# kaspanet/rusty-kaspa

Hardware: NVIDIA H100
Metric: schnorr_sig_verifies_per_sec (higher is better)
Workload: dtype u32 limbs (256-bit modular integer)

## Files before the change

__graft_entry__.py:

```python
import os
import subprocess
import sys

ROOT = os.path.dirname(os.path.abspath(__file__))
CSRC = os.path.join(ROOT, "rusty_kaspa_b200", "csrc")
LIB = os.path.join(ROOT, "rusty_kaspa_b200", "libkgv.so")
NVCC_FLAGS = ["-gencode", "arch=compute_90a,code=sm_90a", "-O3", "-lineinfo", "-std=c++17", "-shared", "-Xcompiler", "-fPIC"]


def _newer(target, sources):
    if not os.path.exists(target):
        return True
    t = os.path.getmtime(target)
    return any(os.path.getmtime(s) > t for s in sources)


def _run(cmd, **kw):
    r = subprocess.run(cmd, capture_output=True, text=True, **kw)
    if r.returncode != 0:
        raise RuntimeError("command failed: %s\n%s\n%s" % (" ".join(cmd), r.stdout[-4000:], r.stderr[-4000:]))
    return r


def build():
    srcs = [os.path.join(d, f) for d, _, fs in os.walk(CSRC) for f in fs] + [os.path.join(ROOT, "include", "kgv.h")]
    units = sorted(s for s in srcs if s.endswith(".cu") or s.endswith(".cpp"))
    if _newer(LIB, srcs):
        nvcc = os.environ.get("NVCC", "nvcc")
        _run([nvcc] + NVCC_FLAGS + ["-o", LIB] + units)
    _run(["make", "-C", os.path.join(ROOT, "oracle")])
    hs = os.path.join(ROOT, "tests", "hostsim")
    for name in ("hostsim_arith", "hostsim_secp", "hostsim_comb", "hostsim_joint", "hostsim_hash", "hostsim_u3072", "hostsim_script"):
        src, out = os.path.join(hs, name + ".cpp"), os.path.join(hs, "lib" + name + ".so")
        if os.path.exists(src) and _newer(out, [src] + srcs):
            _run(["g++", "-O2", "-std=c++17", "-shared", "-fPIC", "-o", out, src])
    sg_src, sg_lib = os.path.join(ROOT, "tools", "simgen", "kgv_simgen.cpp"), os.path.join(ROOT, "tools", "simgen", "libkgv_simgen.so")
    if os.path.exists(sg_src) and _newer(sg_lib, [sg_src]):
        _run(["g++", "-O2", "-std=c++17", "-shared", "-fPIC", "-o", sg_lib, sg_src])
    for name in ("host_mirror_test", "script_engine_mirror_test"):
        cpp_src, cpp_bin = os.path.join(ROOT, "tests", "cpp", name + ".cpp"), os.path.join(ROOT, "tests", "cpp", name)
        if os.path.exists(cpp_src) and _newer(cpp_bin, [cpp_src, LIB, os.path.join(ROOT, "include", "kgv.hpp"), os.path.join(ROOT, "include", "kgv.h")]):
            _run(["g++", "-O2", "-std=c++17", "-o", cpp_bin, cpp_src, "-L" + os.path.join(ROOT, "rusty_kaspa_b200"), "-l:libkgv.so", "-Wl,-rpath,$ORIGIN/../../rusty_kaspa_b200"])
    sys.path.insert(0, ROOT)
    import rusty_kaspa_b200
    from rusty_kaspa_b200 import _lib
    _lib.load()


def smoke():
    import ctypes
    import numpy as np
    sys.path.insert(0, ROOT)
    import rusty_kaspa_b200 as rk
    from rusty_kaspa_b200 import workload as W
    pk, msg, sig, kind = W.schnorr_triples(4096, seed=7, n_keys=256, n_nonces=256, frac_bitflip=0.05, frac_adversarial=0.05)
    ctx = rk.GpuContext(0)
    got = ctx.verify_schnorr_batch(pk, msg, sig)
    ora = ctypes.CDLL(os.path.join(ROOT, "oracle", "libkaspa_oracle.so"))
    ora.ok_secp_init()
    exp = np.zeros(len(pk), dtype=np.uint8)
    vp = lambda a: a.ctypes.data_as(ctypes.c_void_p)
    ora.ok_schnorr_verify_batch(vp(pk), vp(msg), vp(sig), ctypes.c_size_t(len(pk)), vp(exp), 4)
    assert (got == exp).all(), "GPU verdicts differ from the oracle"
    assert (got[kind == 0] == 1).all() and not (got[kind != 0] == 1).any()
    bm = ctx.status_to_bitmap(got)
# ... 43 lines not shown
```

rusty_kaspa_b200/csrc/kgv_internal.h:

```cpp
#pragma once
#include <cuda_runtime.h>
#include <cstdint>
#include <mutex>
#include <string>
#include <thread>
#include <vector>

#ifndef KGV_BLOCK
#define KGV_BLOCK 128
#endif
#ifndef KGV_BLOCKS_PER_SM
#define KGV_BLOCKS_PER_SM 3
#endif

#ifndef KGV_ITEMS
#define KGV_ITEMS 4
#endif

struct kgv_ctx {
  int device = 0;
  cudaStream_t own_stream = nullptr;
  cudaStream_t aux_stream = nullptr;
  cudaEvent_t ev_fork = nullptr, ev_join = nullptr;
  cudaEvent_t ev_time[3] = {};
  cudaEvent_t ev_chunk[32] = {};
  cudaStream_t stream = nullptr;
  uint32_t* gtab = nullptr;
  uint8_t* d_in = nullptr;
  size_t d_in_cap = 0;
  uint8_t* d_out = nullptr;
  size_t d_out_cap = 0;
  uint8_t* d_batch = nullptr;
  size_t d_batch_cap = 0;
  struct PrefetchSlot {
    uint8_t* buf = nullptr;
    size_t cap = 0;
    bool valid = false;
    const void *txs = nullptr, *inputs = nullptr, *outputs = nullptr, *entries = nullptr, *bytes = nullptr;
    size_t n_txs = 0, n_inputs = 0, n_outputs = 0, n_bytes = 0;
    cudaEvent_t done = nullptr;
    std::thread worker;
    int rc = 0;
    std::string err;
  } prefetch[2];
  int prefetch_next = 0;
  cudaEvent_t ev_prefetch = nullptr;
  cudaStream_t copy_stream = nullptr;
  uint8_t* d_scratch = nullptr;
  size_t d_scratch_cap = 0;
  uint8_t* d_work = nullptr;
  size_t d_work_cap = 0;
  uint8_t* d_replay = nullptr;
  size_t d_replay_cap = 0;
  uint8_t* d_keys[2] = {};
  size_t d_keys_cap[2] = {};
  uint8_t* d_mu = nullptr;
  size_t d_mu_cap = 0;
  struct {
    bool valid = false;
    const void *txs = nullptr, *inputs = nullptr, *outputs = nullptr, *bytes = nullptr;
    size_t nt = 0, ni = 0, no = 0, n_blocks = 0;
    size_t o_ids = 0, o_itx = 0, o_otx = 0, o_ent = 0, o_acc = 0, o_txb = 0, o_rng = 0;
    size_t o_src = 0, o_inf = 0, o_apv = 0;
  } last_replay;
  struct kgv_sigcache* sigcache = nullptr;
  struct kgv_comm* shard_comm = nullptr;
  std::vector<uint8_t*> parked;
  uint64_t launches = 0;
  uint32_t last_script_rounds = 0;
  struct {
    size_t n = 0;
    unsigned blocks = 0;
    bool key_cache = false;
    cudaStream_t stream = nullptr;
  } last_verify[2];
  int resident_blocks = 132 * KGV_BLOCKS_PER_SM;
  std::recursive_mutex mu;
  std::string err;
};

int kgv_ptr_is_device(const void* p);
int kgv_malloc(kgv_ctx* ctx, void** p, size_t bytes);
int kgv_reserve(kgv_ctx* ctx, uint8_t** buf, size_t* cap, size_t need);

#include "../../include/kgv.h"
struct kgv_dev_batch {
  const kgv_tx* txs;
  const kgv_input* inputs;
// ... 44 lines not shown
```

rusty_kaspa_b200/csrc/kgv_lib.cu:

```cuda
#include "../../include/kgv.h"
#include "kgv_internal.h"
#include "kgv_verify.cuh"
#include "kgv_lanes.cuh"

#include <cuda_runtime.h>
#include <cstdio>
#include <algorithm>
#include <cstring>
#include <mutex>
#include <string>

using namespace kgv;

struct SmemTab {
  uint32_t* base;
  __device__ __forceinline__ void put(int e, int w, uint32_t v) { base[(e * 16 + w) * KGV_BLOCK] = v; }
  __device__ __forceinline__ uint32_t get(int e, int w) const { return base[(e * 16 + w) * KGV_BLOCK]; }
  __device__ __forceinline__ uint4* chunk(int q) const { return reinterpret_cast<uint4*>(base - threadIdx.x) + q * KGV_BLOCK + threadIdx.x; }
};
__device__ __forceinline__ void stage_fetch(SmemTab& tab, int s, const uint32_t* entry) {
#pragma unroll
  for (int c = 0; c < 4; c++) {
    const uint32_t dst = (uint32_t)__cvta_generic_to_shared(tab.chunk(4 * s + c));
    asm volatile("cp.async.cg.shared.global [%0], [%1], 16;" ::"r"(dst), "l"(entry + 4 * c) : "memory");
// ... 129 lines not shown
      bool eq = true;
      for (int k = 0; k < nw; k++) eq = eq && v[k] == w[k];
      if (eq) break;
    }
    s = (s + 1) & mask;
  }
  const uint32_t act = __activemask(), ball = __ballot_sync(act, won);
  const int lane = threadIdx.x & 31, leader = __ffs(act) - 1;
  uint32_t base = 0;
  if (lane == leader && ball) base = atomicAdd(n_rec, (uint32_t)__popc(ball));
  base = __shfl_sync(act, base, leader);
  if (won) {
    const uint32_t r = base + __popc(ball & ((1u << lane) - 1));
    if (key_form(r + 1, n) != KGV_KEYS_INLINE) {
      rec_rep[r] = (uint32_t)i;
      table[s].rec = r + 1;
    }
  }
  item_slot[i] = s;
}

template <bool ECDSA>
__global__ void __launch_bounds__(KGV_BLOCK, KGV_BLOCKS_PER_SM) k_key_prepare(const uint8_t* __restrict__ pk, size_t n_arg, const uint32_t* __restrict__ n_dev,
                                                                              const uint32_t* __restrict__ rec_rep, const uint32_t* __restrict__ n_rec,
                                                                              uint32_t* __restrict__ recs) {
  const size_t n = n_dev ? (size_t)*n_dev : n_arg;
  const uint32_t r = blockIdx.x * blockDim.x + threadIdx.x;
  const int f = key_form(*n_rec, n);
  if (r >= *n_rec || f == KGV_KEYS_INLINE) return;
  uint32_t w[9];
  key_words<false, ECDSA>(w, pk, rec_rep[r]);
  if (f == KGV_KEYS_COMB) {
    uint32_t* rec = recs + (size_t)r * KGV_KJ_WORDS;
    key_comb_build(rec, ECDSA ? w[8] : 2u, w);
    if (rec[KGV_KC_STATUS] == KGV_ST_VALID) key_joint_build(rec);
  } else key_rec_build(recs + (size_t)r * KGV_KR_WORDS, ECDSA ? w[8] : 2u, w);
}

template <bool ECDSA>
__device__ __forceinline__ void batch_mul(fe& r, const fe& a, const fe& b) {
  if constexpr (ECDSA) sc_mul(r.v, a.v, b.v);
  else fe_mul(r, a, b);
}
template <bool ECDSA, bool ALIGNED, bool INDEXED>
__device__ __forceinline__ void verify_body(const uint8_t* __restrict__ pk, const uint8_t* __restrict__ msg, const uint8_t* __restrict__ sig,
                                            size_t n_arg, uint8_t* __restrict__ status, const uint32_t* __restrict__ gtab,
                                            const uint32_t* __restrict__ index, const uint32_t* __restrict__ n_dev, KeyCacheView kc) {
  extern __shared__ uint32_t smem[];
  const size_t n = (INDEXED && n_dev) ? (size_t)*n_dev : n_arg;
  const size_t total = (size_t)gridDim.x * KGV_BLOCK;
  const size_t tid = (size_t)blockIdx.x * KGV_BLOCK + threadIdx.x;
  SmemTab tab{smem + threadIdx.x};
  fe X[KGV_ITEMS], Y[KGV_ITEMS], RX[KGV_ITEMS], D[KGV_ITEMS], pre[KGV_ITEMS], M[KGV_ITEMS];
  const uint32_t* KR[KGV_ITEMS];
  bool comb = false;
  uint8_t st[KGV_ITEMS];
#pragma unroll 1
  for (size_t base = 0; base < n; base += total * KGV_ITEMS) {
  fe acc;
  fe_set_u32(acc, 1);
  bool any = false;
#pragma unroll 1
  for (int j = 0; j < KGV_ITEMS; j++) {
    size_t i = base + tid + (size_t)j * total;
    st[j] = KGV_ST_INVALID;
    if (i >= n) continue;
    if (INDEXED) i = index[i];
    uint32_t pkw[9], mw[8], sw[16];
    key_words<ALIGNED, ECDSA>(pkw, pk, i);
    load_be32<ALIGNED>(mw, msg + 32 * i);
    load_be32<ALIGNED>(sw, sig + 64 * i);
    load_be32<ALIGNED>(sw + 8, sig + 64 * i + 32);
    const KeySrc key = kc.key_of(i, n);
    fe x, y, rx, d, m;
    uint8_t s1;
    if constexpr (ECDSA) s1 = ecdsa_phase1(x, y, rx.v, d.v, m.v, pkw[8], pkw, mw, sw, key);
    else s1 = schnorr_phase1(x, y, d, rx, pkw, mw, sw, tab, gtab, GLoadDev(), key);
    st[j] = s1;
    if (s1 == KGV_ST_PENDING) {
      X[j] = x; Y[j] = y; RX[j] = rx; D[j] = d;
      if constexpr (ECDSA) { M[j] = m; KR[j] = key.rec; comb = key.comb; }
      pre[j] = acc;
      batch_mul<ECDSA>(acc, acc, d);
      any = true;
    }
  }
  if (any) {
    fe inv;
    if constexpr (ECDSA) sc_inv(inv.v, acc.v);
    else fe_inv(inv, acc);
#pragma unroll 1
    for (int j = KGV_ITEMS - 1; j >= 0; j--) {
      if (st[j] != KGV_ST_PENDING) continue;
      fe di;
      batch_mul<ECDSA>(di, inv, pre[j]);
      batch_mul<ECDSA>(inv, inv, D[j]);
      if constexpr (ECDSA) st[j] = ecdsa_phase2(X[j], Y[j], RX[j].v, di.v, M[j].v, tab, gtab, GLoadDev(), KeySrc{KR[j], comb});
      else st[j] = schnorr_phase2(X[j], Y[j], di, RX[j]);
    }
  }
#pragma unroll 1
  for (int j = 0; j < KGV_ITEMS; j++) {
    size_t i = base + tid + (size_t)j * total;
    if (i < n) status[INDEXED ? index[i] : i] = st[j];
  }
  }
}

template <bool ALIGNED, bool INDEXED>
__global__ void __launch_bounds__(KGV_BLOCK, KGV_BLOCKS_PER_SM)
k_schnorr_verify(const uint8_t* __restrict__ pk, const uint8_t* __restrict__ msg, const uint8_t* __restrict__ sig, size_t n_arg,
                 uint8_t* __restrict__ status, const uint32_t* __restrict__ gtab, const uint32_t* __restrict__ index, const uint32_t* __restrict__ n_dev,
                 KeyCacheView kc) {
  verify_body<false, ALIGNED, INDEXED>(pk, msg, sig, n_arg, status, gtab, index, n_dev, kc);
}
template <bool ALIGNED, bool INDEXED>
__global__ void __launch_bounds__(KGV_BLOCK, KGV_BLOCKS_PER_SM)
k_ecdsa_verify(const uint8_t* __restrict__ pk, const uint8_t* __restrict__ msg, const uint8_t* __restrict__ sig, size_t n_arg,
               uint8_t* __restrict__ status, const uint32_t* __restrict__ gtab, const uint32_t* __restrict__ index, const uint32_t* __restrict__ n_dev,
               KeyCacheView kc) {
  verify_body<true, ALIGNED, INDEXED>(pk, msg, sig, n_arg, status, gtab, index, n_dev, kc);
}
using VerifyKernel = void (*)(const uint8_t*, const uint8_t*, const uint8_t*, size_t, uint8_t*, const uint32_t*, const uint32_t*, const uint32_t*,
                              KeyCacheView);
static const VerifyKernel k_verify[2][2][2] = {
    {{k_schnorr_verify<false, false>, k_schnorr_verify<true, false>}, {k_schnorr_verify<false, true>, k_schnorr_verify<true, true>}},
    {{k_ecdsa_verify<false, false>, k_ecdsa_verify<true, false>}, {k_ecdsa_verify<false, true>, k_ecdsa_verify<true, true>}}};

struct DevTrace {
  uint32_t* out;
  __device__ __forceinline__ void operator()(int stage, const uint32_t* w, int n) const {
    for (int i = 0; i < n && i < 16; i++) out[stage * 16 + i] = w[i];
  }
};
__global__ void __launch_bounds__(KGV_BLOCK, KGV_BLOCKS_PER_SM)
k_schnorr_trace(const uint8_t* __restrict__ pk, const uint8_t* __restrict__ msg, const uint8_t* __restrict__ sig,
                uint8_t* __restrict__ status, const uint32_t* __restrict__ gtab, uint32_t* __restrict__ dbg) {
  extern __shared__ uint32_t smem[];
  if (threadIdx.x != 0 || blockIdx.x != 0) return;
  uint32_t pkw[8], mw[8], sw[16];
  load_be32<false>(pkw, pk);
  load_be32<false>(mw, msg);
  load_be32<false>(sw, sig);
  load_be32<false>(sw + 8, sig + 32);
  SmemTab tab{smem + threadIdx.x};
  status[0] = schnorr_verify_core(pkw, mw, sw, tab, gtab, GLoadDev(), DevTrace{dbg});
}

__global__ void k_selftest(int op, const uint32_t* __restrict__ in, uint32_t* __restrict__ out, int n) {
  int i = blockIdx.x * blockDim.x + threadIdx.x;
  if (i >= n) return;
  uint32_t a[8], b[8], r[16];
#pragma unroll
  for (int k = 0; k < 8; k++) { a[k] = in[i * 16 + k]; b[k] = in[i * 16 + 8 + k]; }
#pragma unroll
  for (int k = 0; k < 16; k++) r[k] = 0;
  fe fa, fb, fr;
// ... 113 lines not shown
    CK(cudaEventCreateWithFlags(&ctx->ev_join, cudaEventDisableTiming));
    CK(cudaMalloc((void**)&ctx->gtab, (size_t)8 * 65536 * 16 * sizeof(uint32_t)));
    k_build_gtab<<<(8 * 65536) / 128, 128, 0, ctx->stream>>>(ctx->gtab);
    CK(cudaGetLastError());
    ctx->launches++;
    const int smem = KGV_BLOCK * 128 * (int)sizeof(uint32_t);
    for (const auto& kind : k_verify)
      for (const auto& form : kind)
        for (VerifyKernel k : form) CK(cudaFuncSetAttribute(k, cudaFuncAttributeMaxDynamicSharedMemorySize, smem));
    int per_sm = 0, sms = 0;
    CK(cudaOccupancyMaxActiveBlocksPerMultiprocessor(&per_sm, k_verify[0][0][1], KGV_BLOCK, smem));
    CK(cudaDeviceGetAttribute(&sms, cudaDevAttrMultiProcessorCount, device));
    ctx->resident_blocks = per_sm * sms > 0 ? per_sm * sms : 132 * KGV_BLOCKS_PER_SM;
    CK(cudaStreamSynchronize(ctx->stream));
    return KGV_OK;
  };
  int rc = body();
  if (rc != KGV_OK) {
    fprintf(stderr, "kgv_create: %s\n", ctx->err.c_str());
    delete ctx;
    return rc;
  }
  *out = ctx;
  return KGV_OK;
}

extern "C" void kgv_destroy(kgv_ctx* ctx) {
  if (!ctx) return;
  cudaSetDevice(ctx->device);
  for (auto& P : ctx->prefetch) if (P.worker.joinable()) P.worker.join();
  if (ctx->copy_stream) cudaStreamSynchronize(ctx->copy_stream);
  cudaStreamSynchronize(ctx->stream);
  if (ctx->gtab) cudaFree(ctx->gtab);
  for (uint8_t* b : {ctx->d_in, ctx->d_out, ctx->d_batch, ctx->prefetch[0].buf, ctx->prefetch[1].buf, ctx->d_scratch, ctx->d_mu, ctx->d_work, ctx->d_replay, ctx->d_keys[0], ctx->d_keys[1]})
    if (b) cudaFree(b);
  for (uint8_t* b : ctx->parked) cudaFree(b);
  for (cudaEvent_t e : ctx->ev_chunk) if (e) cudaEventDestroy(e);
  for (cudaEvent_t e : ctx->ev_time) if (e) cudaEventDestroy(e);
  if (ctx->ev_prefetch) cudaEventDestroy(ctx->ev_prefetch);
  for (auto& P : ctx->prefetch) if (P.done) cudaEventDestroy(P.done);
  if (ctx->copy_stream) cudaStreamDestroy(ctx->copy_stream);
  if (ctx->ev_fork) cudaEventDestroy(ctx->ev_fork);
  if (ctx->ev_join) cudaEventDestroy(ctx->ev_join);
  if (ctx->aux_stream) cudaStreamDestroy(ctx->aux_stream);
  if (ctx->own_stream) cudaStreamDestroy(ctx->own_stream);
  delete ctx;
}

extern "C" int kgv_set_stream(kgv_ctx* ctx, void* cuda_stream) {
  if (!ctx) return KGV_ERR_ARG;
  std::lock_guard<std::recursive_mutex> g(ctx->mu);
  ctx->stream = (cudaStream_t)cuda_stream;
  return KGV_OK;
}

extern "C" int kgv_reset_stream(kgv_ctx* ctx) {
  if (!ctx) return KGV_ERR_ARG;
  std::lock_guard<std::recursive_mutex> g(ctx->mu);
  ctx->stream = ctx->own_stream;
  return KGV_OK;
}

extern "C" int kgv_synchronize(kgv_ctx* ctx) {
  if (!ctx) return KGV_ERR_ARG;
  std::lock_guard<std::recursive_mutex> g(ctx->mu);
  CK(cudaSetDevice(ctx->device));
  CK(cudaStreamSynchronize(ctx->stream));
// ... 20 lines not shown
  const size_t o_rep = (o_item + n * 4 + 255) & ~(size_t)255, o_rec = (o_rep + (size_t)cap * 4 + 255) & ~(size_t)255;
  int rc = kgv_reserve(ctx, &ctx->d_keys[ecdsa], &ctx->d_keys_cap[ecdsa], o_rec + rec_bytes);
  if (rc) return rc;
  uint8_t* K = ctx->d_keys[ecdsa];
  uint32_t* n_rec = (uint32_t*)K;
  KeySlot* table = (KeySlot*)(K + o_tab);
  uint32_t *item_slot = (uint32_t*)(K + o_item), *rec_rep = (uint32_t*)(K + o_rep), *recs = (uint32_t*)(K + o_rec);
  CK(cudaMemsetAsync(K, 0, o_item, st));
  const unsigned gd = (unsigned)((n + 255) / 256);
  const auto dedup = ecdsa ? k_key_dedup<false, true> : aligned ? k_key_dedup<true, false> : k_key_dedup<false, false>;
  dedup<<<gd, 256, 0, st>>>(dpk, n, index, n_dev, table, slots - 1, item_slot, rec_rep, n_rec);
  CK(cudaGetLastError());
  ctx->launches++;
  if (cap) {
    const unsigned gp = (cap + KGV_BLOCK - 1) / KGV_BLOCK;
    const auto prepare = ecdsa ? k_key_prepare<true> : k_key_prepare<false>;
    prepare<<<gp, KGV_BLOCK, 0, st>>>(dpk, n, n_dev, rec_rep, n_rec, recs);
    CK(cudaGetLastError());
    ctx->launches++;
  }
  *kc = KeyCacheView{table, item_slot, recs, n_rec};
  return KGV_OK;
}

int kgv_launch_verify(kgv_ctx* ctx, const uint8_t* dpk, const uint8_t* dmsg, const uint8_t* dsig, size_t n, uint8_t* dst, bool ecdsa,
                      cudaStream_t st, const uint32_t* index, const uint32_t* n_dev) {
  if (n == 0) return KGV_OK;
  if (n >= 0x7FFFFFFFu) return fail_arg(ctx, "verify launch of 2^31 or more items");
  const int smem = KGV_BLOCK * 128 * (int)sizeof(uint32_t);
  size_t want = (n + KGV_BLOCK - 1) / KGV_BLOCK;
  unsigned blocks = (unsigned)(want < (size_t)ctx->resident_blocks ? want : (size_t)ctx->resident_blocks);
  bool aligned = (((uintptr_t)dmsg | (uintptr_t)dsig | (ecdsa ? 0 : (uintptr_t)dpk)) & 31) == 0;
  KeyCacheView kc{};
  const bool key_cache = n > (size_t)ctx->resident_blocks * KGV_BLOCK;
  if (key_cache) {
    int rc = key_cache_launch(ctx, dpk, n, ecdsa, aligned, st, index, n_dev, &kc);
    if (rc) return rc;
  }
  if (!index) {
    auto& lv = ctx->last_verify[ecdsa];
    lv.n = n; lv.blocks = blocks; lv.key_cache = key_cache; lv.stream = st;
  }
  k_verify[ecdsa][index != nullptr][aligned]<<<blocks, KGV_BLOCK, smem, st>>>(dpk, dmsg, dsig, n, dst, ctx->gtab, index, n_dev, kc);
  CK(cudaGetLastError());
  ctx->launches++;
  return KGV_OK;
}

static int verify_common(kgv_ctx* ctx, const uint8_t* pk, size_t pk_stride, const uint8_t* msg, const uint8_t* sig, size_t n,
                         uint8_t* status, bool ecdsa) {
  if (!ctx) return KGV_ERR_ARG;
  std::lock_guard<std::recursive_mutex> g(ctx->mu);
  if (n == 0) return KGV_OK;
  if (!pk || !msg || !sig || !status) return fail_arg(ctx, "null buffer");
  CK(cudaSetDevice(ctx->device));
  int dev = kgv_ptr_is_device(pk);
  if (kgv_ptr_is_device(msg) != dev || kgv_ptr_is_device(sig) != dev || kgv_ptr_is_device(status) != dev)
    return fail_arg(ctx, "all buffers of one call must be host pointers or all device pointers");
  const uint8_t *dpk = pk, *dmsg = msg, *dsig = sig;
  uint8_t* dst = status;
  if (!dev) {
    size_t off_msg = (pk_stride * n + 255) & ~(size_t)255;
    size_t off_sig = off_msg + 32 * n;
    int rc = kgv_reserve(ctx, &ctx->d_in, &ctx->d_in_cap, off_sig + 64 * n);
    if (rc) return rc;
    rc = kgv_reserve(ctx, &ctx->d_out, &ctx->d_out_cap, n);
    if (rc) return rc;
    dpk = ctx->d_in; dmsg = ctx->d_in + off_msg; dsig = ctx->d_in + off_sig; dst = ctx->d_out;
    const size_t chunk = (size_t)ctx->resident_blocks * KGV_BLOCK * KGV_ITEMS;
    if (n >= 2 * chunk && (n + chunk - 1) / chunk <= 32) {
      CK(cudaEventRecord(ctx->ev_fork, ctx->stream));
      CK(cudaStreamWaitEvent(ctx->aux_stream, ctx->ev_fork, 0));
      size_t c = 0;
      for (size_t a = 0; a < n; a += chunk, c++) {
        const size_t m = n - a < chunk ? n - a : chunk;
        if (!ctx->ev_chunk[c]) CK(cudaEventCreateWithFlags(&ctx->ev_chunk[c], cudaEventDisableTiming));
        CK(cudaMemcpyAsync(ctx->d_in + pk_stride * a, pk + pk_stride * a, pk_stride * m, cudaMemcpyHostToDevice, ctx->aux_stream));
        CK(cudaMemcpyAsync(ctx->d_in + off_msg + 32 * a, msg + 32 * a, 32 * m, cudaMemcpyHostToDevice, ctx->aux_stream));
        CK(cudaMemcpyAsync(ctx->d_in + off_sig + 64 * a, sig + 64 * a, 64 * m, cudaMemcpyHostToDevice, ctx->aux_stream));
        CK(cudaEventRecord(ctx->ev_chunk[c], ctx->aux_stream));
        CK(cudaStreamWaitEvent(ctx->stream, ctx->ev_chunk[c], 0));
        int rc2 = kgv_launch_verify(ctx, dpk + pk_stride * a, dmsg + 32 * a, dsig + 64 * a, m, dst + a, ecdsa, ctx->stream);
        if (rc2) return rc2;
      }
      CK(cudaMemcpyAsync(status, dst, n, cudaMemcpyDeviceToHost, ctx->stream));
      CK(cudaStreamSynchronize(ctx->stream));
      return KGV_OK;
    }
    CK(cudaMemcpyAsync(ctx->d_in, pk, pk_stride * n, cudaMemcpyHostToDevice, ctx->stream));
    CK(cudaMemcpyAsync(ctx->d_in + off_msg, msg, 32 * n, cudaMemcpyHostToDevice, ctx->stream));
    CK(cudaMemcpyAsync(ctx->d_in + off_sig, sig, 64 * n, cudaMemcpyHostToDevice, ctx->stream));
  }
  {
    int rc = kgv_launch_verify(ctx, dpk, dmsg, dsig, n, dst, ecdsa, ctx->stream);
    if (rc) return rc;
  }
  if (!dev) {
    CK(cudaMemcpyAsync(status, dst, n, cudaMemcpyDeviceToHost, ctx->stream));
    CK(cudaStreamSynchronize(ctx->stream));
  }
  return KGV_OK;
}
// ... 124 lines not shown
```

rusty_kaspa_b200/csrc/kgv_secp.cuh:

```cuda
#pragma once
#include "kgv_arith.cuh"

namespace kgv {

#define KGV_N_LIMBS {0xD0364141u, 0xBFD25E8Cu, 0xAF48A03Bu, 0xBAAEDCE6u, 0xFFFFFFFEu, 0xFFFFFFFFu, 0xFFFFFFFFu, 0xFFFFFFFFu}
#define KGV_BETA_LIMBS {0x719501EEu, 0xC1396C28u, 0x12F58995u, 0x9CF04975u, 0xAC3434E9u, 0x6E64479Eu, 0x657C0710u, 0x7AE96A2Bu}
#define KGV_G1_LIMBS {0x45DBB031u, 0xE893209Au, 0x71E8CA7Fu, 0x3DAA8A14u, 0x9284EB15u, 0xE86C90E4u, 0xA7D46BCDu, 0x3086D221u}
#define KGV_G2_LIMBS {0x8AC47F71u, 0x1571B4AEu, 0x9DF506C6u, 0x221208ACu, 0x0ABFE4C4u, 0x6F547FA9u, 0x010E8828u, 0xE4437ED6u}
#define KGV_A1_LIMBS {0x9284EB15u, 0xE86C90E4u, 0xA7D46BCDu, 0x3086D221u, 0u}
#define KGV_MB1_LIMBS {0x0ABFE4C3u, 0x6F547FA9u, 0x010E8828u, 0xE4437ED6u, 0u}
#define KGV_A2_LIMBS {0x9D44CFD8u, 0x57C1108Du, 0xA8E2F3F6u, 0x14CA50F7u, 1u}

struct gej {
  fe x, y, z;
  bool inf;
};

struct NoTrace {
  KGV_HD void operator()(int , const uint32_t* , int ) const {}
};

KGV_HD bool sc_ge_n(const uint32_t* a) {
  const uint32_t n[8] = KGV_N_LIMBS;
  return !lt8(a, n);
// ... 328 lines not shown
  gej_h o = gej_point_call(r, bx, by, 0);
  r = o.r;
  if (hout) *hout = o.h;
}
#else
KGV_HD void gej_double_n(gej& r, int n) {
  if (r.inf) return;
  for (int i = 0; i < n; i++) gej_double_body(r);
}
KGV_HD void gej_add_ge(gej& r, const fe& bx, const fe& by, fe* hout = nullptr) {
  if (gej_add_ge_body(r, bx, by, hout)) {
    if (hout) fe_dbl(*hout, r.y);
    gej_double_n(r, 1);
  }
}
#endif
KGV_HD void gej_double(gej& r) { gej_double_n(r, 1); }

KGV_HD bool ge_lift_x(fe& y, const fe& x, bool odd) {
  fe t, c;
  fe_sqr(t, x);
  fe_mul(t, t, x);
  fe_set_u32(c, 7);
  fe_add(c, t, c);
  if (!fe_sqrt(y, c)) return false;
  fe_normalize(y);
  if (((y.v[0] & 1u) != 0) != odd) {
    fe_neg(y, y);
    fe_normalize(y);
  }
  return true;
}

template <class Tab>
KGV_HD void build_odd_table(Tab& tab, fe& zs, const fe& px, const fe& py) {
  gej d;
  d.x = px; d.y = py; fe_set_u32(d.z, 1); d.inf = false;
  gej_double(d);
  fe zd2, zd3;
  fe_sqr(zd2, d.z);
  fe_mul(zd3, zd2, d.z);
  gej t;
  fe_mul(t.x, px, zd2);
  fe_mul(t.y, py, zd3);
  fe_set_u32(t.z, 1);
  t.inf = false;
  fe H[7];
#pragma unroll
  for (int w = 0; w < 8; w++) { tab.put(0, w, t.x.v[w]); tab.put(0, 8 + w, t.y.v[w]); }
#pragma unroll
  for (int j = 1; j < 8; j++) {
    gej_add_ge(t, d.x, d.y, &H[j - 1]);
#pragma unroll
    for (int w = 0; w < 8; w++) { tab.put(j, w, t.x.v[w]); tab.put(j, 8 + w, t.y.v[w]); }
  }
  fe acc = H[6];
#pragma unroll
  for (int j = 6; j >= 0; j--) {
    if (j < 6) fe_mul(acc, acc, H[j]);
    fe a2, a3, ex, ey;
    fe_sqr(a2, acc);
    fe_mul(a3, a2, acc);
#pragma unroll
    for (int w = 0; w < 8; w++) { ex.v[w] = tab.get(j, w); ey.v[w] = tab.get(j, 8 + w); }
    fe_mul(ex, ex, a2);
    fe_mul(ey, ey, a3);
#pragma unroll
    for (int w = 0; w < 8; w++) { tab.put(j, w, ex.v[w]); tab.put(j, 8 + w, ey.v[w]); }
  }
  fe_mul(zs, t.z, d.z);
}

template <class Tab, class GLoad, class Trace = NoTrace>
KGV_HD void ecmult_double(gej& R, const fe& zs, const uint32_t* kP, const uint32_t* kG, Tab& tab, const uint32_t* gtab, GLoad gload,
                          Trace trace = Trace()) {
  const fe beta = {KGV_BETA_LIMBS};
  uint32_t m1[5], m2[5], h1[5], h2[5];
  bool neg1, neg2, fix1, fix2;
  glv_split(m1, neg1, m2, neg2, kP);
  recode_signed_odd(h1, fix1, m1);
  recode_signed_odd(h2, fix2, m2);
  trace(10, m1, 5); trace(11, m2, 5);
  { uint32_t f[4] = {neg1, neg2, fix1, fix2}; trace(12, f, 4); }
  trace(13, zs.v, 8);
  { uint32_t e0[16]; for (int w = 0; w < 16; w++) e0[w] = tab.get(7, w); trace(14, e0, 16); }
  fe zs2, zs3;
  fe_sqr(zs2, zs);
  fe_mul(zs3, zs2, zs);

  R.inf = true;
  fe_set_zero(R.x); fe_set_zero(R.y); fe_set_zero(R.z);
  for (int i = 32; i >= 0; i--) {
// ... 229 lines not shown
```

rusty_kaspa_b200/csrc/kgv_verify.cuh:

```cuda
#pragma once
#include "kgv_secp.cuh"
#include "kgv_sha256.cuh"

namespace kgv {

enum : uint8_t { KGV_ST_INVALID = 0, KGV_ST_VALID = 1, KGV_ST_PK_PARSE = 2, KGV_ST_SIG_PARSE = 3 };

KGV_HD bool fe_words_lt_p(const uint32_t* v) {
  const uint32_t p[8] = {KGV_P0, KGV_P1, 0xFFFFFFFFu, 0xFFFFFFFFu, 0xFFFFFFFFu, 0xFFFFFFFFu, 0xFFFFFFFFu, 0xFFFFFFFFu};
  return lt8(v, p);
}

#define KGV_ST_PENDING 0xFFu

KGV_HD bool key_lift(fe& x, fe& y, uint32_t tag, const uint32_t* pkw) {
  if (tag != 2u && tag != 3u) return false;
  limbs_from_be_words(x.v, pkw);
  if (!fe_words_lt_p(x.v)) return false;
  return ge_lift_x(y, x, tag == 3u);
}

#define KGV_KR_ZS 128
#define KGV_KR_STATUS 136
#define KGV_KR_WORDS 140
// ... 25 lines not shown
KGV_HD void fe_st(uint32_t* p, const fe& x) {
#ifdef __CUDA_ARCH__
  reinterpret_cast<uint4*>(p)[0] = make_uint4(x.v[0], x.v[1], x.v[2], x.v[3]);
  reinterpret_cast<uint4*>(p)[1] = make_uint4(x.v[4], x.v[5], x.v[6], x.v[7]);
#else
  for (int w = 0; w < 8; w++) p[w] = x.v[w];
#endif
}
template <class Tab>
KGV_HD void key_rec_load(Tab& tab, fe& zs, const uint32_t* rec) {
#pragma unroll 1
  for (int e = 0; e < 8; e++) {
    uint32_t w[16];
#pragma unroll
    for (int q = 0; q < 4; q++) ldg128(w + 4 * q, rec + 16 * e + 4 * q);
#pragma unroll
    for (int q = 0; q < 16; q++) tab.put(e, q, w[q]);
  }
  ldg128(zs.v, rec + KGV_KR_ZS);
  ldg128(zs.v + 4, rec + KGV_KR_ZS + 4);
}
KGV_HD void key_rec_build(uint32_t* rec, uint32_t tag, const uint32_t* pkw) {
  fe x, y, zs;
  uint8_t st = KGV_ST_PK_PARSE;
  if (key_lift(x, y, tag, pkw)) {
    RecTab tab{rec};
    build_odd_table(tab, zs, x, y);
#pragma unroll
    for (int w = 0; w < 8; w++) rec[KGV_KR_ZS + w] = zs.v[w];
    st = KGV_ST_VALID;
  }
  rec[KGV_KR_STATUS] = st;
}
KGV_HD void key_comb_build(uint32_t* rec, uint32_t tag, const uint32_t* pkw) {
  fe x, y;
  uint8_t st = KGV_ST_PK_PARSE;
  if (key_lift(x, y, tag, pkw)) {
    gej b;
    b.x = x; b.y = y; fe_set_u32(b.z, 1); b.inf = false;
    fe zs[4], pre[4], inv;
#pragma unroll 1
    for (int t = 0; t < 4; t++) {
      if (t) gej_double_n(b, 32);
      RecTab tab{rec + 128 * t};
      fe z;
      build_odd_table(tab, z, b.x, b.y);
      fe_mul(zs[t], z, b.z);
      if (t) fe_mul(pre[t], pre[t - 1], zs[t]);
      else pre[0] = zs[0];
    }
    fe_inv(inv, pre[3]);
#pragma unroll 1
    for (int t = 3; t >= 0; t--) {
      fe zi, zi2, zi3;
      if (t) {
        fe_mul(zi, inv, pre[t - 1]);
        fe_mul(inv, inv, zs[t]);
      } else {
        zi = inv;
      }
      fe_sqr(zi2, zi);
      fe_mul(zi3, zi2, zi);
#pragma unroll 1
      for (int e = 0; e < 8; e++) {
        uint32_t* en = rec + 16 * (8 * t + e);
        fe ex, ey;
        fe_ld(ex, en);
        fe_ld(ey, en + 8);
        fe_mul(ex, ex, zi2);
        fe_mul(ey, ey, zi3);
        fe_st(en, ex);
        fe_st(en + 8, ey);
      }
    }
    st = KGV_ST_VALID;
  }
  rec[KGV_KC_STATUS] = st;
}

KGV_HD void key_joint_build(uint32_t* rec) {
  const fe beta = {KGV_BETA_LIMBS};
  uint32_t* jt = rec + KGV_KJ_JOINT;
#pragma unroll 1
  for (int t = 0; t < 4; t++) {
#pragma unroll 1
    for (int j = 0; j < 4; j++) {
      fe bx;
      fe_ld(bx, rec + 16 * (8 * t + j));
      fe_mul(bx, bx, beta);
      fe_st(jt + 16 * (32 * t + 3 - j), bx);
    }
  }
  fe acc;
  fe_set_u32(acc, 1);
#pragma unroll 1
  for (int ta = 0; ta < 16; ta++) {
    const int t = ta >> 2, a = ta & 3;
// ... 76 lines not shown
template <class Tab, class GLoad, class Trace = NoTrace>
KGV_HD uint8_t schnorr_phase1(fe& X, fe& Y, fe& zt, fe& rx, const uint32_t* pkw, const uint32_t* mw, const uint32_t* sigw, Tab& tab,
                              const uint32_t* gtab, GLoad gload, const KeySrc& key, Trace trace = Trace()) {
  fe px, py;
  if (key.rec) {
    if (!key_rec_valid(key)) return KGV_ST_PK_PARSE;
  } else {
    limbs_from_be_words(px.v, pkw);
    if (!fe_words_lt_p(px.v)) return KGV_ST_PK_PARSE;
    trace(1, px.v, 8);
    if (!ge_lift_x(py, px, false)) return KGV_ST_PK_PARSE;
    trace(2, py.v, 8);
  }
  limbs_from_be_words(rx.v, sigw);
  if (!fe_words_lt_p(rx.v)) return KGV_ST_INVALID;
  uint32_t s[8], e[8], k[8], ew[8];
  limbs_from_be_words(s, sigw + 8);
  if (sc_ge_n(s)) return KGV_ST_INVALID;
  bip340_challenge(ew, sigw, pkw, mw);
#pragma unroll
  for (int i = 0; i < 8; i++) e[7 - i] = ew[i];
  sc_reduce_once(e);
  sc_neg(k, e);
  trace(3, e, 8); trace(4, k, 8); trace(5, s, 8);
  gej R;
  ecmult_key(R, zt, key, px, py, k, s, tab, gtab, gload, trace);
  { uint32_t f[1] = {R.inf}; trace(18, f, 1); }
  if (R.inf) return KGV_ST_INVALID;
  trace(19, R.x.v, 8); trace(20, R.y.v, 8); trace(21, R.z.v, 8);
  X = R.x;
  Y = R.y;
  return KGV_ST_PENDING;
}
template <class Trace = NoTrace>
KGV_HD uint8_t schnorr_phase2(const fe& X, const fe& Y, const fe& zi, const fe& rx, Trace trace = Trace()) {
  fe zi2, ax, ay;
  fe_sqr(zi2, zi);
  fe_mul(ax, X, zi2);
  fe_mul(ay, Y, zi2);
  fe_mul(ay, ay, zi);
  fe_normalize(ay);
  fe_normalize(ax);
  trace(22, ax.v, 8); trace(23, ay.v, 8);
  if (ay.v[0] & 1u) return KGV_ST_INVALID;
  bool eq = true;
#pragma unroll
  for (int i = 0; i < 8; i++) eq = eq && (ax.v[i] == rx.v[i]);
  return eq ? KGV_ST_VALID : KGV_ST_INVALID;
}
template <class Tab, class GLoad, class Trace = NoTrace>
KGV_HD uint8_t schnorr_verify_core(const uint32_t* pkw, const uint32_t* mw, const uint32_t* sigw, Tab& tab, const uint32_t* gtab,
                                   GLoad gload, Trace trace = Trace(), KeySrc key = KeySrc{nullptr, false}) {
  fe X, Y, zt, rx, zi;
  uint8_t st = schnorr_phase1(X, Y, zt, rx, pkw, mw, sigw, tab, gtab, gload, key, trace);
  if (st != KGV_ST_PENDING) return st;
  fe_inv(zi, zt);
  return schnorr_phase2(X, Y, zi, rx, trace);
}

KGV_HD uint8_t ecdsa_phase1(fe& qx, fe& qy, uint32_t* r, uint32_t* s, uint32_t* m, uint32_t tag, const uint32_t* pkw, const uint32_t* mw,
                            const uint32_t* sigw, const KeySrc& key) {
  if (key.rec) {
    if (!key_rec_valid(key)) return KGV_ST_PK_PARSE;
  } else if (!key_lift(qx, qy, tag, pkw)) {
    return KGV_ST_PK_PARSE;
  }
  limbs_from_be_words(r, sigw);
  limbs_from_be_words(s, sigw + 8);
  if (sc_ge_n(r) || sc_ge_n(s)) return KGV_ST_SIG_PARSE;
  limbs_from_be_words(m, mw);
  sc_reduce_once(m);
  if (sc_is_high(s)) return KGV_ST_INVALID;
  if (is_zero8(r) || is_zero8(s)) return KGV_ST_INVALID;
  return KGV_ST_PENDING;
}
template <class Tab, class GLoad>
KGV_HD uint8_t ecdsa_phase2(const fe& qx, const fe& qy, const uint32_t* r, const uint32_t* sn, const uint32_t* m, Tab& tab, const uint32_t* gtab,
                            GLoad gload, const KeySrc& key) {
  uint32_t u1[8], u2[8];
  sc_mul(u1, sn, m);
  sc_mul(u2, sn, r);
  gej R;
  fe zt;
  ecmult_key(R, zt, key, qx, qy, u2, u1, tab, gtab, gload);
  if (R.inf) return KGV_ST_INVALID;
  fe zt2, t, rf;
  fe_sqr(zt2, zt);
#pragma unroll
  for (int i = 0; i < 8; i++) rf.v[i] = r[i];
  fe_mul(t, rf, zt2);
// ... 64 lines not shown
```

Before: 61.87 million.

## Check Schnorr x in Jacobian form and spill batch-inversion state to global scratch

The Schnorr x-coordinate check now compares rx·Z² against X in Jacobian coordinates before any inversion, so phase 2 only needs Y and Z⁻¹ to test y-parity, and invalid signatures skip the batched inversion. The fixed per-thread KGV_ITEMS register arrays are replaced by a grid-stride loop that writes pending field elements to a global scratch buffer, so one Montgomery batch inversion covers all of a thread's items, with a direct single-item path when n fits in one wave. Key comb tables get an odd-multiple count template parameter, instantiated at 4. The change trades register pressure and extra inversions for global-memory traffic through L2 on the pending state.

```diff
diff --git a/__graft_entry__.py b/__graft_entry__.py
--- a/__graft_entry__.py
+++ b/__graft_entry__.py
@@ -30,7 +30,7 @@
         _run([nvcc] + NVCC_FLAGS + ["-o", LIB] + units)
     _run(["make", "-C", os.path.join(ROOT, "oracle")])
     hs = os.path.join(ROOT, "tests", "hostsim")
-    for name in ("hostsim_arith", "hostsim_secp", "hostsim_comb", "hostsim_joint", "hostsim_hash", "hostsim_u3072", "hostsim_script"):
+    for name in ("hostsim_arith", "hostsim_secp", "hostsim_comb", "hostsim_joint", "hostsim_comb4", "hostsim_hash", "hostsim_u3072", "hostsim_script"):
         src, out = os.path.join(hs, name + ".cpp"), os.path.join(hs, "lib" + name + ".so")
         if os.path.exists(src) and _newer(out, [src] + srcs):
             _run(["g++", "-O2", "-std=c++17", "-shared", "-fPIC", "-o", out, src])
diff --git a/rusty_kaspa_b200/csrc/kgv_internal.h b/rusty_kaspa_b200/csrc/kgv_internal.h
--- a/rusty_kaspa_b200/csrc/kgv_internal.h
+++ b/rusty_kaspa_b200/csrc/kgv_internal.h
@@ -13,9 +13,7 @@
 #define KGV_BLOCKS_PER_SM 3
 #endif
 
-#ifndef KGV_ITEMS
-#define KGV_ITEMS 4
-#endif
+#define KGV_UPLOAD_CHUNK_ITEMS 4
 
 struct kgv_ctx {
   int device = 0;
@@ -54,6 +52,8 @@
   size_t d_replay_cap = 0;
   uint8_t* d_keys[2] = {};
   size_t d_keys_cap[2] = {};
+  uint8_t* d_pend[2] = {};
+  size_t d_pend_cap[2] = {};
   uint8_t* d_mu = nullptr;
   size_t d_mu_cap = 0;
   struct {
diff --git a/rusty_kaspa_b200/csrc/kgv_lib.cu b/rusty_kaspa_b200/csrc/kgv_lib.cu
--- a/rusty_kaspa_b200/csrc/kgv_lib.cu
+++ b/rusty_kaspa_b200/csrc/kgv_lib.cu
@@ -185,7 +185,7 @@
   key_words<false, ECDSA>(w, pk, rec_rep[r]);
   if (f == KGV_KEYS_COMB) {
     uint32_t* rec = recs + (size_t)r * KGV_KJ_WORDS;
-    key_comb_build(rec, ECDSA ? w[8] : 2u, w);
+    key_comb_build<4>(rec, ECDSA ? w[8] : 2u, w);
     if (rec[KGV_KC_STATUS] == KGV_ST_VALID) key_joint_build(rec);
   } else key_rec_build(recs + (size_t)r * KGV_KR_WORDS, ECDSA ? w[8] : 2u, w);
 }
@@ -195,68 +195,114 @@
   if constexpr (ECDSA) sc_mul(r.v, a.v, b.v);
   else fe_mul(r, a, b);
 }
+#define KGV_PEND_FIELDS_SCHNORR 3
+#define KGV_PEND_FIELDS_ECDSA 6
+template <bool ECDSA>
+struct Pending {
+  static constexpr int FIELDS = ECDSA ? KGV_PEND_FIELDS_ECDSA : KGV_PEND_FIELDS_SCHNORR, PRE = FIELDS - (ECDSA ? 3 : 1);
+  fe f[FIELDS];
+  const uint32_t* rec;
+  __device__ __forceinline__ int stored() const { return ECDSA && rec ? 4 : FIELDS; }
+};
+struct PendScratch {
+  uint4* base;
+  size_t pitch;
+  __device__ __forceinline__ void put(int f, size_t p, const fe& x) const {
+    __stcg(base + (2 * f) * pitch + p, make_uint4(x.v[0], x.v[1], x.v[2], x.v[3]));
+    __stcg(base + (2 * f + 1) * pitch + p, make_uint4(x.v[4], x.v[5], x.v[6], x.v[7]));
+  }
+  __device__ __forceinline__ void get(int f, size_t p, fe& x) const {
+    const uint4 a = __ldcg(base + (2 * f) * pitch + p), b = __ldcg(base + (2 * f + 1) * pitch + p);
+    x.v[0] = a.x; x.v[1] = a.y; x.v[2] = a.z; x.v[3] = a.w; x.v[4] = b.x; x.v[5] = b.y; x.v[6] = b.z; x.v[7] = b.w;
+  }
+};
+template <bool ECDSA, bool ALIGNED>
+__device__ __forceinline__ uint8_t verify_phase1(Pending<ECDSA>& q, size_t i, size_t n, const uint8_t* __restrict__ pk,
+                                                 const uint8_t* __restrict__ msg, const uint8_t* __restrict__ sig, SmemTab& tab,
+                                                 const uint32_t* __restrict__ gtab, const KeyCacheView& kc) {
+  uint32_t pkw[9], mw[8], sw[16];
+  key_words<ALIGNED, ECDSA>(pkw, pk, i);
+  load_be32<ALIGNED>(mw, msg + 32 * i);
+  load_be32<ALIGNED>(sw, sig + 64 * i);
+  load_be32<ALIGNED>(sw + 8, sig + 64 * i + 32);
+  const KeySrc key = kc.key_of(i, n);
+  if constexpr (ECDSA) {
+    q.rec = key.rec;
+    return ecdsa_phase1(q.f[4], q.f[5], q.f[0].v, q.f[1].v, q.f[2].v, pkw[8], pkw, mw, sw, key);
+  } else {
+    fe x, r;
+    const uint8_t s1 = schnorr_phase1(x, q.f[0], q.f[1], r, pkw, mw, sw, tab, gtab, GLoadDev(), key);
+    if (s1 == KGV_ST_PENDING && !schnorr_x_matches(x, q.f[1], r)) return KGV_ST_INVALID;
+    return s1;
+  }
+}
+template <bool ECDSA>
+__device__ __forceinline__ uint8_t verify_phase2(const Pending<ECDSA>& q, const fe& di, size_t i, size_t n, SmemTab& tab,
+                                                 const uint32_t* __restrict__ gtab, const KeyCacheView& kc) {
+  if constexpr (ECDSA) return ecdsa_phase2(q.f[4], q.f[5], q.f[0].v, di.v, q.f[2].v, tab, gtab, GLoadDev(), kc.key_of(i, n));
+  else return schnorr_phase2(q.f[0], di);
+}
 template <bool ECDSA, bool ALIGNED, bool INDEXED>
 __device__ __forceinline__ void verify_body(const uint8_t* __restrict__ pk, const uint8_t* __restrict__ msg, const uint8_t* __restrict__ sig,
                                             size_t n_arg, uint8_t* __restrict__ status, const uint32_t* __restrict__ gtab,
-                                            const uint32_t* __restrict__ index, const uint32_t* __restrict__ n_dev, KeyCacheView kc) {
+                                            const uint32_t* __restrict__ index, const uint32_t* __restrict__ n_dev, KeyCacheView kc,
+                                            uint4* __restrict__ pend_base) {
   extern __shared__ uint32_t smem[];
   const size_t n = (INDEXED && n_dev) ? (size_t)*n_dev : n_arg;
   const size_t total = (size_t)gridDim.x * KGV_BLOCK;
   const size_t tid = (size_t)blockIdx.x * KGV_BLOCK + threadIdx.x;
+  if (tid >= n) return;
   SmemTab tab{smem + threadIdx.x};
-  fe X[KGV_ITEMS], Y[KGV_ITEMS], RX[KGV_ITEMS], D[KGV_ITEMS], pre[KGV_ITEMS], M[KGV_ITEMS];
-  const uint32_t* KR[KGV_ITEMS];
-  bool comb = false;
-  uint8_t st[KGV_ITEMS];
-#pragma unroll 1
-  for (size_t base = 0; base < n; base += total * KGV_ITEMS) {
+  Pending<ECDSA> q;
+  constexpr int PRE = Pending<ECDSA>::PRE;
+  if (n <= total) {
+    const size_t i = INDEXED ? index[tid] : tid;
+    uint8_t st = verify_phase1<ECDSA, ALIGNED>(q, i, n, pk, msg, sig, tab, gtab, kc);
+    if (st == KGV_ST_PENDING) {
+      fe di;
+      if constexpr (ECDSA) sc_inv(di.v, q.f[1].v);
+      else fe_inv(di, q.f[1]);
+      st = verify_phase2<ECDSA>(q, di, i, n, tab, gtab, kc);
+    }
+    status[i] = st;
+    return;
+  }
+  const PendScratch pend{pend_base, n_arg};
   fe acc;
   fe_set_u32(acc, 1);
   bool any = false;
 #pragma unroll 1
-  for (int j = 0; j < KGV_ITEMS; j++) {
-    size_t i = base + tid + (size_t)j * total;
-    st[j] = KGV_ST_INVALID;
-    if (i >= n) continue;
-    if (INDEXED) i = index[i];
-    uint32_t pkw[9], mw[8], sw[16];
-    key_words<ALIGNED, ECDSA>(pkw, pk, i);
-    load_be32<ALIGNED>(mw, msg + 32 * i);
-    load_be32<ALIGNED>(sw, sig + 64 * i);
-    load_be32<ALIGNED>(sw + 8, sig + 64 * i + 32);
-    const KeySrc key = kc.key_of(i, n);
-    fe x, y, rx, d, m;
-    uint8_t s1;
-    if constexpr (ECDSA) s1 = ecdsa_phase1(x, y, rx.v, d.v, m.v, pkw[8], pkw, mw, sw, key);
-    else s1 = schnorr_phase1(x, y, d, rx, pkw, mw, sw, tab, gtab, GLoadDev(), key);
-    st[j] = s1;
+  for (size_t p = tid; p < n; p += total) {
+    const size_t i = INDEXED ? index[p] : p;
+    const uint8_t s1 = verify_phase1<ECDSA, ALIGNED>(q, i, n, pk, msg, sig, tab, gtab, kc);
     if (s1 == KGV_ST_PENDING) {
-      X[j] = x; Y[j] = y; RX[j] = rx; D[j] = d;
-      if constexpr (ECDSA) { M[j] = m; KR[j] = key.rec; comb = key.comb; }
-      pre[j] = acc;
-      batch_mul<ECDSA>(acc, acc, d);
+      q.f[PRE] = acc;
+      batch_mul<ECDSA>(acc, acc, q.f[1]);
       any = true;
+#pragma unroll
+      for (int f = 0; f < Pending<ECDSA>::FIELDS; f++)
+        if (f < q.stored()) pend.put(f, p, q.f[f]);
     }
-  }
-  if (any) {
-    fe inv;
-    if constexpr (ECDSA) sc_inv(inv.v, acc.v);
-    else fe_inv(inv, acc);
+    status[i] = s1;
+  }
+  if (!any) return;
+  fe inv;
+  if constexpr (ECDSA) sc_inv(inv.v, acc.v);
+  else fe_inv(inv, acc);
 #pragma unroll 1
-    for (int j = KGV_ITEMS - 1; j >= 0; j--) {
-      if (st[j] != KGV_ST_PENDING) continue;
+  for (size_t p = tid + (n - 1 - tid) / total * total;; p -= total) {
+    const size_t i = INDEXED ? index[p] : p;
+    if (status[i] == KGV_ST_PENDING) {
+      if constexpr (ECDSA) q.rec = kc.key_of(i, n).rec;
+#pragma unroll
+      for (int f = 0; f < Pending<ECDSA>::FIELDS; f++)
+        if (f < q.stored()) pend.get(f, p, q.f[f]);
       fe di;
-      batch_mul<ECDSA>(di, inv, pre[j]);
-      batch_mul<ECDSA>(inv, inv, D[j]);
-      if constexpr (ECDSA) st[j] = ecdsa_phase2(X[j], Y[j], RX[j].v, di.v, M[j].v, tab, gtab, GLoadDev(), KeySrc{KR[j], comb});
-      else st[j] = schnorr_phase2(X[j], Y[j], di, RX[j]);
+      batch_mul<ECDSA>(di, inv, q.f[PRE]);
+      batch_mul<ECDSA>(inv, inv, q.f[1]);
+      status[i] = verify_phase2<ECDSA>(q, di, i, n, tab, gtab, kc);
     }
-  }
-#pragma unroll 1
-  for (int j = 0; j < KGV_ITEMS; j++) {
-    size_t i = base + tid + (size_t)j * total;
-    if (i < n) status[INDEXED ? index[i] : i] = st[j];
-  }
+    if (p < total) break;
   }
 }
 
@@ -264,18 +310,18 @@
 __global__ void __launch_bounds__(KGV_BLOCK, KGV_BLOCKS_PER_SM)
 k_schnorr_verify(const uint8_t* __restrict__ pk, const uint8_t* __restrict__ msg, const uint8_t* __restrict__ sig, size_t n_arg,
                  uint8_t* __restrict__ status, const uint32_t* __restrict__ gtab, const uint32_t* __restrict__ index, const uint32_t* __restrict__ n_dev,
-                 KeyCacheView kc) {
-  verify_body<false, ALIGNED, INDEXED>(pk, msg, sig, n_arg, status, gtab, index, n_dev, kc);
+                 KeyCacheView kc, uint4* __restrict__ pend) {
+  verify_body<false, ALIGNED, INDEXED>(pk, msg, sig, n_arg, status, gtab, index, n_dev, kc, pend);
 }
 template <bool ALIGNED, bool INDEXED>
 __global__ void __launch_bounds__(KGV_BLOCK, KGV_BLOCKS_PER_SM)
 k_ecdsa_verify(const uint8_t* __restrict__ pk, const uint8_t* __restrict__ msg, const uint8_t* __restrict__ sig, size_t n_arg,
                uint8_t* __restrict__ status, const uint32_t* __restrict__ gtab, const uint32_t* __restrict__ index, const uint32_t* __restrict__ n_dev,
-               KeyCacheView kc) {
-  verify_body<true, ALIGNED, INDEXED>(pk, msg, sig, n_arg, status, gtab, index, n_dev, kc);
+               KeyCacheView kc, uint4* __restrict__ pend) {
+  verify_body<true, ALIGNED, INDEXED>(pk, msg, sig, n_arg, status, gtab, index, n_dev, kc, pend);
 }
 using VerifyKernel = void (*)(const uint8_t*, const uint8_t*, const uint8_t*, size_t, uint8_t*, const uint32_t*, const uint32_t*, const uint32_t*,
-                              KeyCacheView);
+                              KeyCacheView, uint4*);
 static const VerifyKernel k_verify[2][2][2] = {
     {{k_schnorr_verify<false, false>, k_schnorr_verify<true, false>}, {k_schnorr_verify<false, true>, k_schnorr_verify<true, true>}},
     {{k_ecdsa_verify<false, false>, k_ecdsa_verify<true, false>}, {k_ecdsa_verify<false, true>, k_ecdsa_verify<true, true>}}};
@@ -455,7 +501,7 @@
   if (ctx->copy_stream) cudaStreamSynchronize(ctx->copy_stream);
   cudaStreamSynchronize(ctx->stream);
   if (ctx->gtab) cudaFree(ctx->gtab);
-  for (uint8_t* b : {ctx->d_in, ctx->d_out, ctx->d_batch, ctx->prefetch[0].buf, ctx->prefetch[1].buf, ctx->d_scratch, ctx->d_mu, ctx->d_work, ctx->d_replay, ctx->d_keys[0], ctx->d_keys[1]})
+  for (uint8_t* b : {ctx->d_in, ctx->d_out, ctx->d_batch, ctx->prefetch[0].buf, ctx->prefetch[1].buf, ctx->d_scratch, ctx->d_mu, ctx->d_work, ctx->d_replay, ctx->d_keys[0], ctx->d_keys[1], ctx->d_pend[0], ctx->d_pend[1]})
     if (b) cudaFree(b);
   for (uint8_t* b : ctx->parked) cudaFree(b);
   for (cudaEvent_t e : ctx->ev_chunk) if (e) cudaEventDestroy(e);
@@ -542,16 +588,19 @@
   unsigned blocks = (unsigned)(want < (size_t)ctx->resident_blocks ? want : (size_t)ctx->resident_blocks);
   bool aligned = (((uintptr_t)dmsg | (uintptr_t)dsig | (ecdsa ? 0 : (uintptr_t)dpk)) & 31) == 0;
   KeyCacheView kc{};
-  const bool key_cache = n > (size_t)ctx->resident_blocks * KGV_BLOCK;
-  if (key_cache) {
+  const bool several = n > (size_t)ctx->resident_blocks * KGV_BLOCK;
+  if (several) {
     int rc = key_cache_launch(ctx, dpk, n, ecdsa, aligned, st, index, n_dev, &kc);
     if (rc) return rc;
+    rc = kgv_reserve(ctx, &ctx->d_pend[ecdsa], &ctx->d_pend_cap[ecdsa], n * 32 * (ecdsa ? KGV_PEND_FIELDS_ECDSA : KGV_PEND_FIELDS_SCHNORR));
+    if (rc) return rc;
   }
   if (!index) {
     auto& lv = ctx->last_verify[ecdsa];
-    lv.n = n; lv.blocks = blocks; lv.key_cache = key_cache; lv.stream = st;
-  }
-  k_verify[ecdsa][index != nullptr][aligned]<<<blocks, KGV_BLOCK, smem, st>>>(dpk, dmsg, dsig, n, dst, ctx->gtab, index, n_dev, kc);
+    lv.n = n; lv.blocks = blocks; lv.key_cache = several; lv.stream = st;
+  }
+  k_verify[ecdsa][index != nullptr][aligned]<<<blocks, KGV_BLOCK, smem, st>>>(dpk, dmsg, dsig, n, dst, ctx->gtab, index, n_dev, kc,
+                                                                               several ? (uint4*)ctx->d_pend[ecdsa] : nullptr);
   CK(cudaGetLastError());
   ctx->launches++;
   return KGV_OK;
@@ -577,7 +626,7 @@
     rc = kgv_reserve(ctx, &ctx->d_out, &ctx->d_out_cap, n);
     if (rc) return rc;
     dpk = ctx->d_in; dmsg = ctx->d_in + off_msg; dsig = ctx->d_in + off_sig; dst = ctx->d_out;
-    const size_t chunk = (size_t)ctx->resident_blocks * KGV_BLOCK * KGV_ITEMS;
+    const size_t chunk = (size_t)ctx->resident_blocks * KGV_BLOCK * KGV_UPLOAD_CHUNK_ITEMS;
     if (n >= 2 * chunk && (n + chunk - 1) / chunk <= 32) {
       CK(cudaEventRecord(ctx->ev_fork, ctx->stream));
       CK(cudaStreamWaitEvent(ctx->aux_stream, ctx->ev_fork, 0));
diff --git a/rusty_kaspa_b200/csrc/kgv_secp.cuh b/rusty_kaspa_b200/csrc/kgv_secp.cuh
--- a/rusty_kaspa_b200/csrc/kgv_secp.cuh
+++ b/rusty_kaspa_b200/csrc/kgv_secp.cuh
@@ -384,8 +384,9 @@
   return true;
 }
 
-template <class Tab>
+template <int ODD = 8, class Tab>
 KGV_HD void build_odd_table(Tab& tab, fe& zs, const fe& px, const fe& py) {
+  static_assert(ODD >= 2 && ODD <= 8, "odd multiples {1,3,..,2*ODD-1}");
   gej d;
   d.x = px; d.y = py; fe_set_u32(d.z, 1); d.inf = false;
   gej_double(d);
@@ -397,19 +398,19 @@
   fe_mul(t.y, py, zd3);
   fe_set_u32(t.z, 1);
   t.inf = false;
-  fe H[7];
+  fe H[ODD - 1];
 #pragma unroll
   for (int w = 0; w < 8; w++) { tab.put(0, w, t.x.v[w]); tab.put(0, 8 + w, t.y.v[w]); }
 #pragma unroll
-  for (int j = 1; j < 8; j++) {
+  for (int j = 1; j < ODD; j++) {
     gej_add_ge(t, d.x, d.y, &H[j - 1]);
 #pragma unroll
     for (int w = 0; w < 8; w++) { tab.put(j, w, t.x.v[w]); tab.put(j, 8 + w, t.y.v[w]); }
   }
-  fe acc = H[6];
-#pragma unroll
-  for (int j = 6; j >= 0; j--) {
-    if (j < 6) fe_mul(acc, acc, H[j]);
+  fe acc = H[ODD - 2];
+#pragma unroll
+  for (int j = ODD - 2; j >= 0; j--) {
+    if (j < ODD - 2) fe_mul(acc, acc, H[j]);
     fe a2, a3, ex, ey;
     fe_sqr(a2, acc);
     fe_mul(a3, a2, acc);
diff --git a/rusty_kaspa_b200/csrc/kgv_verify.cuh b/rusty_kaspa_b200/csrc/kgv_verify.cuh
--- a/rusty_kaspa_b200/csrc/kgv_verify.cuh
+++ b/rusty_kaspa_b200/csrc/kgv_verify.cuh
@@ -81,6 +81,7 @@
   }
   rec[KGV_KR_STATUS] = st;
 }
+template <int ODD = 8>
 KGV_HD void key_comb_build(uint32_t* rec, uint32_t tag, const uint32_t* pkw) {
   fe x, y;
   uint8_t st = KGV_ST_PK_PARSE;
@@ -93,7 +94,7 @@
       if (t) gej_double_n(b, 32);
       RecTab tab{rec + 128 * t};
       fe z;
-      build_odd_table(tab, z, b.x, b.y);
+      build_odd_table<ODD>(tab, z, b.x, b.y);
       fe_mul(zs[t], z, b.z);
       if (t) fe_mul(pre[t], pre[t - 1], zs[t]);
       else pre[0] = zs[0];
@@ -111,7 +112,7 @@
       fe_sqr(zi2, zi);
       fe_mul(zi3, zi2, zi);
 #pragma unroll 1
-      for (int e = 0; e < 8; e++) {
+      for (int e = 0; e < ODD; e++) {
         uint32_t* en = rec + 16 * (8 * t + e);
         fe ex, ey;
         fe_ld(ex, en);
@@ -254,21 +255,19 @@
   Y = R.y;
   return KGV_ST_PENDING;
 }
-template <class Trace = NoTrace>
-KGV_HD uint8_t schnorr_phase2(const fe& X, const fe& Y, const fe& zi, const fe& rx, Trace trace = Trace()) {
-  fe zi2, ax, ay;
-  fe_sqr(zi2, zi);
-  fe_mul(ax, X, zi2);
-  fe_mul(ay, Y, zi2);
-  fe_mul(ay, ay, zi);
+KGV_HD bool schnorr_x_matches(const fe& X, const fe& zt, const fe& rx) {
+  fe zt2, t;
+  fe_sqr(zt2, zt);
+  fe_mul(t, rx, zt2);
+  return fe_equal(t, X);
+}
+KGV_HD uint8_t schnorr_phase2(const fe& Y, const fe& zi) {
+  fe zi3, ay;
+  fe_sqr(zi3, zi);
+  fe_mul(zi3, zi3, zi);
+  fe_mul(ay, Y, zi3);
   fe_normalize(ay);
-  fe_normalize(ax);
-  trace(22, ax.v, 8); trace(23, ay.v, 8);
-  if (ay.v[0] & 1u) return KGV_ST_INVALID;
-  bool eq = true;
-#pragma unroll
-  for (int i = 0; i < 8; i++) eq = eq && (ax.v[i] == rx.v[i]);
-  return eq ? KGV_ST_VALID : KGV_ST_INVALID;
+  return (ay.v[0] & 1u) ? KGV_ST_INVALID : KGV_ST_VALID;
 }
 template <class Tab, class GLoad, class Trace = NoTrace>
 KGV_HD uint8_t schnorr_verify_core(const uint32_t* pkw, const uint32_t* mw, const uint32_t* sigw, Tab& tab, const uint32_t* gtab,
@@ -277,7 +276,18 @@
   uint8_t st = schnorr_phase1(X, Y, zt, rx, pkw, mw, sigw, tab, gtab, gload, key, trace);
   if (st != KGV_ST_PENDING) return st;
   fe_inv(zi, zt);
-  return schnorr_phase2(X, Y, zi, rx, trace);
+  {
+    fe zi2, ax, ay;
+    fe_sqr(zi2, zi);
+    fe_mul(ax, X, zi2);
+    fe_mul(ay, Y, zi2);
+    fe_mul(ay, ay, zi);
+    fe_normalize(ax);
+    fe_normalize(ay);
+    trace(22, ax.v, 8); trace(23, ay.v, 8);
+  }
+  if (!schnorr_x_matches(X, zt, rx)) return KGV_ST_INVALID;
+  return schnorr_phase2(Y, zi);
 }
 
 KGV_HD uint8_t ecdsa_phase1(fe& qx, fe& qy, uint32_t* r, uint32_t* s, uint32_t* m, uint32_t tag, const uint32_t* pkw, const uint32_t* mw,
```

Measured after the change: 65.44 million (median of 6 runs). 5.8% higher.
